# THUDM/GCC

Measured on AMD Instinct MI355X. Metric: sampled-subgraphs/sec, higher is better.
Workload: dtype f32

## Files before the change

### gcc_amd/csrc/posemb.hip

```cpp
#include <mutex>
#include "host_common.h"
#include <type_traits>

namespace {

constexpr int kJMax = GCC_POSEMB_LDS_MAX;
#ifndef GCC_POSEMB_SMALL_T
#define GCC_POSEMB_SMALL_T 256
#endif
constexpr int kSmallT = GCC_POSEMB_SMALL_T;
constexpr int kJSmall = 64;

constexpr int kMaxViews = GCC_POSEMB_MAX_VIEWS;
struct PosView {
    const int32_t *node_off, *row_ptr, *col_idx;
    float *pos, *evals, *raw;
};
struct PosMulti {
    PosView v[kMaxViews];
    int32_t nviews, B, hidden;
    uint64_t seed;
    int32_t *status;
    long long *ticks;
};
// ... 1994 lines not shown
    const int rp0 = a.row_ptr[n0], nnz = a.row_ptr[n0 + n] - rp0;
    const bool csr_lds = nnz <= kCsrCap && nnz < 65536 && n < ldv;
    if (csr_lds) {
        for (int e = tid; e < nnz; e += kKThreads) ccol[e] = (uint16_t)(a.col_idx[rp0 + e] - n0);
        for (int r = tid; r <= n; r += kKThreads) crow[r] = (uint16_t)(a.row_ptr[n0 + r] - rp0);
    }
    __syncthreads();
    const int nl = nlong < kMaxLong ? nlong : kMaxLong;
    const bool long_overflow = nlong > kMaxLong;

    auto orth = [&](int ncols, int hcol) {
        for (int pass = 0; pass < 2; ++pass) {
            for (int i = 2 * wv_id; i < ncols; i += 2 * kKWaves) {
                const float *va = V + (int64_t)i * ldv;
                const bool two = i + 1 < ncols;
                const float *vb = two ? va + ldv : va;
                float a0 = 0.f, a1 = 0.f, b0 = 0.f, b1 = 0.f;
                for (int r = lane; r < n; r += 256) {
                    const int r1 = r + 64, r2 = r + 128, r3 = r + 192;
                    const float x0 = va[r], y0 = vb[r];
                    const float x1 = r1 < n ? va[r1] : 0.f, y1 = r1 < n ? vb[r1] : 0.f;
                    const float x2 = r2 < n ? va[r2] : 0.f, y2 = r2 < n ? vb[r2] : 0.f;
                    const float x3 = r3 < n ? va[r3] : 0.f, y3 = r3 < n ? vb[r3] : 0.f;
                    const float w0 = w[r], w1 = r1 < n ? w[r1] : 0.f, w2 = r2 < n ? w[r2] : 0.f, w3 = r3 < n ? w[r3] : 0.f;
                    a0 = fmaf(x0, w0, a0); a1 = fmaf(x1, w1, a1); a0 = fmaf(x2, w2, a0); a1 = fmaf(x3, w3, a1);
                    b0 = fmaf(y0, w0, b0); b1 = fmaf(y1, w1, b1); b0 = fmaf(y2, w2, b0); b1 = fmaf(y3, w3, b1);
                }
                const float sa = wave_sum(a0 + a1), sb = wave_sum(b0 + b1);
                if (lane == 0) {
                    hbuf[i] = sa;
                    if (two) hbuf[i + 1] = sb;
                }
            }
            __syncthreads();
            if (hcol >= 0 && tid < ncols) H[tid * kM + hcol] += hbuf[tid];
            for (int r = tid; r < n; r += kKThreads) {
                float a0 = w[r], a1 = 0.f, a2 = 0.f, a3 = 0.f;
                int i = 0;
                for (; i + 8 <= ncols; i += 8) {
                    const float v0 = V[(int64_t)i * ldv + r], v1 = V[(int64_t)(i + 1) * ldv + r];
                    const float v2 = V[(int64_t)(i + 2) * ldv + r], v3 = V[(int64_t)(i + 3) * ldv + r];
                    const float v4 = V[(int64_t)(i + 4) * ldv + r], v5 = V[(int64_t)(i + 5) * ldv + r];
                    const float v6 = V[(int64_t)(i + 6) * ldv + r], v7 = V[(int64_t)(i + 7) * ldv + r];
                    a0 = fmaf(-v0, hbuf[i], a0); a1 = fmaf(-v1, hbuf[i + 1], a1);
                    a2 = fmaf(-v2, hbuf[i + 2], a2); a3 = fmaf(-v3, hbuf[i + 3], a3);
                    a0 = fmaf(-v4, hbuf[i + 4], a0); a1 = fmaf(-v5, hbuf[i + 5], a1);
                    a2 = fmaf(-v6, hbuf[i + 6], a2); a3 = fmaf(-v7, hbuf[i + 7], a3);
                }
                for (; i + 4 <= ncols; i += 4) {
                    a0 = fmaf(-V[(int64_t)i * ldv + r], hbuf[i], a0);
                    a1 = fmaf(-V[(int64_t)(i + 1) * ldv + r], hbuf[i + 1], a1);
                    a2 = fmaf(-V[(int64_t)(i + 2) * ldv + r], hbuf[i + 2], a2);
                    a3 = fmaf(-V[(int64_t)(i + 3) * ldv + r], hbuf[i + 3], a3);
                }
                for (; i < ncols; ++i) a0 = fmaf(-V[(int64_t)i * ldv + r], hbuf[i], a0);
                w[r] = (a0 + a1) + (a2 + a3);
            }
            __syncthreads();
        }
    };

    int j = 0, steps = 0, cycle = 0;
    for (; cycle < kMaxCycles; ++cycle) {
        for (; j < kM; ++j, ++steps) {
            for (int r = tid; r < n; r += kKThreads) {
                const int beg = csr_lds ? (int)crow[r] : a.row_ptr[n0 + r] - rp0;
                const int end = csr_lds ? (int)crow[r + 1] : a.row_ptr[n0 + r + 1] - rp0;
                if (end - beg > kLongDeg && !long_overflow) continue;
                float s = 0.f;
                if (csr_lds) for (int e = beg; e < end; ++e) s += x[ccol[e]];
                else for (int e = beg; e < end; ++e) s += x[a.col_idx[rp0 + e] - n0];
                w[r] = s * dinv[r];
            }
            if (!long_overflow) {
                for (int i = wv_id; i < nl; i += kKWaves) {
                    const int r = longrows[i];
                    const int beg = csr_lds ? (int)crow[r] : a.row_ptr[n0 + r] - rp0;
                    const int end = csr_lds ? (int)crow[r + 1] : a.row_ptr[n0 + r + 1] - rp0;
                    float s = 0.f;
                    if (csr_lds) for (int e = beg + lane; e < end; e += 64) s += x[ccol[e]];
                    else for (int e = beg + lane; e < end; e += 64) s += x[a.col_idx[rp0 + e] - n0];
                    s = wave_sum(s);
                    if (lane == 0) w[r] = s * dinv[r];
                }
            }
            __syncthreads();
            orth(j + 1, j);
            float s2 = 0.f;
            for (int r = tid; r < n; r += kKThreads) s2 = fmaf(w[r], w[r], s2);
            float beta = sqrtf(block_sum(s2, red));
            if (beta < 1e-6f) {
                for (int r = tid; r < n; r += kKThreads) {
                    uint32_t rnd[4];
                    philox4x32_10((uint32_t)r, (uint32_t)(steps + 1), (uint32_t)gb, 0x9E0B5EEDu,
                                  (uint32_t)a.seed, (uint32_t)(a.seed >> 32), rnd);
                    w[r] = (float)(rnd[0] >> 8) * (1.0f / 16777216.0f) - 0.5f;
                }
                __syncthreads();
                orth(j + 1, -1);
                float s3 = 0.f;
                for (int r = tid; r < n; r += kKThreads) s3 = fmaf(w[r], w[r], s3);
                nrm = sqrtf(block_sum(s3, red));
                beta = 0.f;
            } else {
                nrm = beta;
            }
            if (tid == 0) H[(j + 1) * kM + j] = beta;
            for (int r = tid; r < n; r += kKThreads) {
                const float vn = w[r] / nrm;
                V[(int64_t)(j + 1) * ldv + r] = vn;
                x[r] = vn * dinv[r];
            }
            __syncthreads();
        }
        PHASE_TICK(0);
        for (int i = tid; i < kM * lda; i += kKThreads) {
            const int r = i / lda, c = i - r * lda;
            float v = 0.f;
            if (c < kM) v = r <= c ? H[r * kM + c] : H[c * kM + r];
            Aj[i] = v;
        }
        __syncthreads();
        tridiagonalize<1, kKThreads, 2>(Aj, lda, kM, tw);
        eig_top_values<kKThreads, kVecCap>(tw, kM, keep, es);
        const bool ritz_failed = eig_top_vectors<1, kKThreads>(Aj, lda, kM, keep, tw, es,
                                                               (uint32_t)a.seed ^ ((uint32_t)gb * 0x9E3779B1u) ^ (uint32_t)cycle,
                                                               nullptr, tick_);
        PHASE_TICK(1);
        if (tid < kM) {
            theta[tid] = tid < keep ? es.lamv[tid] : -2.f;
            sel[tid] = tid < keep ? tid : kM;
        }
        if (tid == 0) { done = 1; flag = ritz_failed ? 2 : 0; }
        __syncthreads();
        const float beta_m = H[kM * kM + (kM - 1)];
        if (tid < k) {
            const float res = fabsf(beta_m * Yj[(kM - 1) * lda + tid]);
            if (res > kRitzTol) done = 0;
            if (res > 10.f * kRitzTol) flag = 2;
        }
        __syncthreads();
        const bool finished = done != 0 || cycle == kMaxCycles - 1;
#ifdef GCC_AMD_HIPEMU
        if (getenv("GCC_POSEMB_DEBUG") && tid == 0) {
            float worst = 0.f; int nbad = 0;
            for (int i = 0; i < kM; ++i) if (sel[i] < k) { const float rs = fabsf(beta_m * Yj[(kM - 1) * lda + i]); worst = rs > worst ? rs : worst; nbad += rs > kRitzTol; }
            fprintf(stderr, "kry b=%d n=%d cycle=%d worst=%.2e nbad=%d theta_k=%.4f\n", b, n, cycle + 1, worst, nbad, 0.f);
        }
#endif
        if (finished && done == 0 && flag == 2 && tid == 0) {
            atomicOr(a.status, (int32_t)GCC_STATUS_POSEMB_NOT_CONVERGED);
            if (atomicAdd(a.status + 4, 1) == 0) { a.status[5] = gb; a.status[6] = kClsKrylov; a.status[7] = n; a.status[8] = -1; a.status[9] = n; }
        }
        if (finished && done == 0 && tid == 0) atomicAdd(a.status + 3, 1);
        const int nout = finished ? k : keep;
        if (tid < kM) {
            const int t = finished ? k - 1 - sel[tid] : sel[tid];
            if (t >= 0 && t < nout) colsrc[t] = tid;
        }
        __syncthreads();
        if (!finished) {
            const int nchunk = (nout + 7) >> 3;
            for (int task = tid; task < n * nchunk; task += kKThreads) {
                const int ch = task / n, r = task - ch * n;
                float acc[8] = {0.f, 0.f, 0.f, 0.f, 0.f, 0.f, 0.f, 0.f};
                int src[8];
#pragma unroll
                for (int u = 0; u < 8; ++u) src[u] = colsrc[min(8 * ch + u, nout - 1)];
                for (int c = 0; c < kM; ++c) {
                    const float v = V[(int64_t)c * ldv + r];
#pragma unroll
                    for (int u = 0; u < 8; ++u) acc[u] = fmaf(v, Yj[c * lda + src[u]], acc[u]);
                }
#pragma unroll
                for (int u = 0; u < 8; ++u)
                    if (8 * ch + u < nout) Valt[(int64_t)(8 * ch + u) * ldv + r] = acc[u];
            }
            for (int r = tid; r < n; r += kKThreads) Valt[(int64_t)keep * ldv + r] = V[(int64_t)kM * ldv + r];
            for (int i = tid; i < (kM + 1) * kM; i += kKThreads) H[i] = 0.f;
            __syncthreads();
            if (tid < kM && sel[tid] < keep) H[sel[tid] * kM + sel[tid]] = theta[tid];
            __syncthreads();
            float *tmp = V; V = Valt; Valt = tmp;
            j = keep;
            PHASE_TICK(2);
            continue;
        }
        float *rawout = a.raw ? a.raw : a.pos;
        const int nchunk = (k + 7) >> 3;
        for (int task = tid; task < n * nchunk; task += kKThreads) {
            const int ch = task / n, r = task - ch * n;
            float acc[8] = {0.f, 0.f, 0.f, 0.f, 0.f, 0.f, 0.f, 0.f};
            int src[8];
#pragma unroll
            for (int u = 0; u < 8; ++u) src[u] = colsrc[min(8 * ch + u, k - 1)];
            for (int c = 0; c < kM; ++c) {
                const float v = V[(int64_t)c * ldv + r];
#pragma unroll
                for (int u = 0; u < 8; ++u) acc[u] = fmaf(v, Yj[c * lda + src[u]], acc[u]);
            }
            float *ro = rawout + (int64_t)(n0 + r) * a.hidden + 8 * ch;
#pragma unroll
            for (int u = 0; u < 8; ++u)
                if (8 * ch + u < k) ro[u] = acc[u];
        }
        __syncthreads();
        for (int r = tid; r < n; r += kKThreads) {
            const float *ro = rawout + (int64_t)(n0 + r) * a.hidden;
            float *po = a.pos + (int64_t)(n0 + r) * a.hidden;
            float s2 = 0.f;
            for (int c = 0; c < k; ++c) s2 = fmaf(ro[c], ro[c], s2);
            const float inv = s2 > 0.f ? 1.0f / sqrtf(s2) : 1.0f;
            for (int c = 0; c < a.hidden; ++c) {
                const float v = c < k ? ro[c] : 0.f;
                po[c] = v * inv;
                if (a.raw) a.raw[(int64_t)(n0 + r) * a.hidden + c] = v;
            }
        }
        if (a.evals && tid < kM && sel[tid] < k) a.evals[(int64_t)b * a.hidden + (k - 1 - sel[tid])] = theta[tid];
        if (a.evals) for (int c = k + tid; c < a.hidden; c += kKThreads) a.evals[(int64_t)b * a.hidden + c] = 0.f;
        break;
    }
    PHASE_TICK(3);
    if (tid == 0) {
        atomicMax(a.status + 1, cycle + 1);
        atomicAdd(a.status + 2, steps);
    }
    }
}


constexpr int kChP = 64;
constexpr int kChPWide = 64, kChPNarrow = 32;
#ifndef GCC_POSEMB_CH_NARROW_WANT
#define GCC_POSEMB_CH_NARROW_WANT 20
#endif
constexpr int kChNarrowWant = GCC_POSEMB_CH_NARROW_WANT;
constexpr int kChNarrowGuards = 8;
#ifndef GCC_POSEMB_CH_THREADS
#define GCC_POSEMB_CH_THREADS 1024
#endif
constexpr int kChThreads = GCC_POSEMB_CH_THREADS;
static_assert(kChThreads % 64 == 0 && kNodeMax % kChThreads == 0 && kChThreads >= 256 && kChThreads <= 1024, "block-class workgroup size");
constexpr int kChRowsPerThread = kNodeMax / kChThreads;
#if defined(GCC_AMD_HIPEMU) || GCC_POSEMB_CH_THREADS > 512
#define GCC_CHEB_REG_CAP
#else
#define GCC_CHEB_REG_CAP __attribute__((amdgpu_waves_per_eu(GCC_POSEMB_CH_THREADS / 256 + 1)))
#endif
constexpr int kChCsrCap = 12288;
#ifndef GCC_POSEMB_CH_LONGDEG
#define GCC_POSEMB_CH_LONGDEG 32
#endif
constexpr int kChLongDeg = GCC_POSEMB_CH_LONGDEG;
constexpr int kChSlabFloats = 4096;
constexpr int kChMaxChunks = kChSlabFloats / 32;
constexpr int kChMaxLong = kChMaxChunks / 2;
constexpr int kChRounds = 16;
constexpr int kChMaxRitz = 5;
constexpr float kChTol = 2e-5f;
constexpr double kChShift = 1e-8;
constexpr float kChAmpLog = 12.9f;
constexpr int kChBw = 32;

struct LdsYes { static constexpr bool value = true; };
struct LdsNo { static constexpr bool value = false; };

constexpr int64_t kChBufFloats = (int64_t)kNodeMax * kChP;
struct ChebArgs {
    PosMulti m;
    PosHead hd;
    float *xws;
    uint32_t *tabs;
};

template <int P>
struct ChebRitzLds {
    static constexpr int Ldy = P + 1;
    static constexpr int Lf = 0;
    static constexpr int Af = Lf + P * Ldy;
    static constexpr int Y = Af + P * Ldy;
    static constexpr int tri = Y + P * Ldy;
    static constexpr int lu = tri + tri_head_floats(P, P * Ldy, kChThreads);
    static constexpr int bytes = (int)sizeof(float) * lu + tri_lu_bytes(P, kChBw);
};
template <int P>
struct ChebDenseLds {
    static constexpr int G = 0, K = G + P * P, Li = K + P * P;
    static constexpr int bytes = (Li + P * P) * (int)sizeof(double);
};
struct ChebLds {
    static constexpr int crow = 0;
    static constexpr int ccol = crow + (int)sizeof(uint16_t) * (kNodeMax + 8);
    static constexpr int scale = ccol + (int)sizeof(uint16_t) * kChCsrCap;
    static constexpr int slab = scale + (int)sizeof(float) * kNodeMax;
    static constexpr int region = slab + (int)sizeof(float) * kChSlabFloats;
    static constexpr int dense_bytes = ChebDenseLds<kChP>::bytes;
    static constexpr int ritz_pad = kChP * (int)sizeof(float);
    static constexpr int ritz_bytes = ChebRitzLds<kChP>::bytes + ritz_pad;
    static constexpr int region_bytes = ritz_bytes > dense_bytes ? ritz_bytes : dense_bytes;
    static constexpr int bytes = region + region_bytes;
    static_assert(region_bytes >= kNodeMax * kDeflNodeBytes, "the deflation tables overlay the region of the dense matrices");
};

__global__ __launch_bounds__(kChThreads) GCC_CHEB_REG_CAP void posemb_cheb_kernel(ChebArgs ca)
{
    DYN_SMEM(smem);
    __shared__ EigShared es;
    __shared__ float theta[kChP], resid[kChP], dsc[kChP];
    __shared__ double dscd[kChP];
    __shared__ int longrow[kChMaxLong], longfirst[kChMaxLong + 1];
    __shared__ int chunk_beg[kChMaxChunks + 1];
    __shared__ uint8_t chunk_row[kChMaxChunks], rowx[kNodeMax];
    __shared__ int sh_clen, sh_long_t;
    __shared__ int wsum[kChThreads / 64 + 1];
    __shared__ int sh_item, sh_tot[3], sh_nlong, sh_nchunk, sh_fail;
    __shared__ int colsrc[64];
    constexpr int kCls = kClsCheb;
    const PosMulti &m = ca.m;
    const PosHead &hd = ca.hd;
    constexpr int kNW = kChThreads / 64;
    uint16_t *crow = (uint16_t *)(smem + ChebLds::crow);
    uint16_t *ccol = (uint16_t *)(smem + ChebLds::ccol);
    float *scale = (float *)(smem + ChebLds::scale);
    float *slab = (float *)(smem + ChebLds::slab);
    unsigned char *region = smem + ChebLds::region;
    for (;;) {
    __syncthreads();
    if (threadIdx.x == 0) sh_item = atomicAdd(hd.next + kCls, 1);
    __syncthreads();
    if (sh_item >= hd.count[kCls]) return;
    uint32_t tid_ = threadIdx.x;
    opaque_u32(tid_);
    const int tid = (int)tid_, lane = tid & 63, wv = tid >> 6;
    const int gb = hd.list[(int64_t)kCls * hd.T + sh_item] & kItemMask;
    PosArgs a;
    int b;
    item_args(m, gb, a, b);
    const int n0 = a.node_off[b], n = a.node_off[b + 1] - n0;
#ifdef GCC_POSEMB_ABLATE_CHEB
    continue;
#endif
    const int k = min(min(n - 2, a.hidden), kMaxVec);
    long long tick_ = m.ticks ? device_ticks() : 0;
    if (m.ticks && tid == 0) atomicAdd((unsigned long long *)&m.ticks[kCls * 16 + 15], 1ull);
    const int32_t *rp = a.row_ptr + n0;
    float *XA0 = ca.xws + (int64_t)blockIdx.x * 3 * kChBufFloats, *XB0 = XA0 + kChBufFloats, *XC0 = XB0 + kChBufFloats;

    Defl d;
    defl_bind(d, region, kNodeMax);
    for (int i = tid; i < n; i += kChThreads) defl_init_node(d, i, rp, a.col_idx, n0);
    if (tid == 0) { sh_fail = 0; sh_nlong = 0; sh_nchunk = 0; }
    __syncthreads();
    for (int i = tid; i < n; i += kChThreads) defl_count_node(d, i, rp, a.col_idx, n0, hd.use_stalks != 0);
    __syncthreads();
    for (int p = tid; p < n; p += kChThreads) defl_order_node(d, p, rp, a.col_idx, n0);
    __syncthreads();
    defl_prefix_block<kChThreads>(d, n, sh_tot, (int *)slab);
    const int nr = sh_tot[0], z = sh_tot[1], zp = sh_tot[2];
    for (int i = tid; i < n; i += kChThreads) {
        if (d.ridx[i] == kNone) continue;
        const int di = rp[i + 1] - rp[i];
        const int pi = d.par[i];
        float sc = 1.0f / sqrtf((float)(di < 1 ? 1 : di));
        if (pi != (int)kNone && d.tcnt[pi] >= 2) {
            sc = sqrtf((float)d.tcnt[pi]);
        } else {
            const int h = d.phub[pi != (int)kNone ? pi : i];
            if (h != (int)kNone && d.pcnt[h] >= 2) sc = pi != (int)kNone ? 1.0f / sqrtf((float)d.pcnt[h]) : sqrtf(0.5f * (float)d.pcnt[h]);
        }
        scale[d.ridx[i]] = sc;
    }
    for (int r = tid; r <= nr; r += kChThreads) crow[r] = 0;
    __syncthreads();
    for (int i = wv; i < n; i += kNW) {
        if (d.ridx[i] == kNone) continue;
        int c = 0;
        for (int e0 = rp[i]; e0 < rp[i + 1]; e0 += 64) {
            const int e = e0 + lane;
            const bool keep = e < rp[i + 1] && d.ridx[a.col_idx[e] - n0] != kNone;
            c += __popcll(wave_ballot(keep));
        }
        if (lane == 0) crow[d.ridx[i] + 1] = (uint16_t)(c > 65535 ? 65535 : c);
    }
    __syncthreads();
    {
        const int r0 = kChRowsPerThread * tid;
        int c[kChRowsPerThread], own = 0;
#pragma unroll
        for (int u = 0; u < kChRowsPerThread; ++u) { c[u] = r0 + u < nr ? (int)crow[r0 + u + 1] : 0; own += c[u]; }
        int incl = wave_scan_incl(own);
        if (lane == 63) wsum[wv] = incl;
        __syncthreads();
        int base = 0;
        for (int q = 0; q < wv; ++q) base += wsum[q];
        incl += base - own;
        __syncthreads();
#pragma unroll
        for (int u = 0; u < kChRowsPerThread; ++u) {
            incl += c[u];
            if (r0 + u < nr) {
                if (incl > kChCsrCap) sh_fail = 1;
                crow[r0 + u + 1] = (uint16_t)(incl > 65535 ? 65535 : incl);
            }
        }
    }
    __syncthreads();
    if (!sh_fail) {
        for (int i = wv; i < n; i += kNW) {
            if (d.ridx[i] == kNone) continue;
            int at = (int)crow[d.ridx[i]];
            for (int e0 = rp[i]; e0 < rp[i + 1]; e0 += 64) {
                const int e = e0 + lane;
                const int rj = e < rp[i + 1] ? (int)d.ridx[a.col_idx[e] - n0] : (int)kNone;
                const unsigned long long mk = wave_ballot(rj != (int)kNone);
                if (rj != (int)kNone) ccol[at + __popcll(mk & lanemask_lt())] = (uint16_t)rj;
                at += __popcll(mk);
            }
        }
    }
    __syncthreads();
    uint16_t *xrec = (uint16_t *)(ca.tabs + (int64_t)blockIdx.x * kTabFloats);
    for (int v = tid; v < n; v += kChThreads) defl_record(d, v, rp, a.col_idx, n0, xrec + 4 * v);
    __syncthreads();
    PHASE_TICK(0);
    bool failed = sh_fail != 0;
    auto build_chunks = [&](int slots) {
        constexpr int R = kChRowsPerThread;
        const int r0 = R * tid;
        int len[R];
#pragma unroll
        for (int u = 0; u < R; ++u) len[u] = (r0 + u < nr && !failed) ? (int)crow[r0 + u + 1] - (int)crow[r0 + u] : 0;
        auto block_scan = [&](int v, int &total) -> int {
            int incl = wave_scan_incl(v);
            if (lane == 63) wsum[wv] = incl;
            __syncthreads();
            int base = 0, tot = 0;
            for (int q = 0; q < kNW; ++q) { if (q < wv) base += wsum[q]; tot += wsum[q]; }
            __syncthreads();
            total = tot;
            return incl - v + base;
        };
        int T = kChLongDeg, nl = 0, x = 0;
        for (;;) {
            int own = 0;
#pragma unroll
            for (int u = 0; u < R; ++u) own += len[u] > T ? 1 : 0;
            x = block_scan(own, nl);
            if (nl <= slots / 2) break;
            T *= 2;
        }
        int own = 0, total = 0;
#pragma unroll
        for (int u = 0; u < R; ++u) own += len[u] > T ? len[u] : 0;
        (void)block_scan(own, total);
        int clen = nl ? (total + (slots - nl) - 1) / (slots - nl) : 8;
        clen = clen < 8 ? 8 : (clen + 3) & ~3;
        own = 0;
#pragma unroll
        for (int u = 0; u < R; ++u) own += len[u] > T ? (len[u] + clen - 1) / clen : 0;
        int nc = 0;
        int fx = block_scan(own, nc);
#pragma unroll
        for (int u = 0; u < R; ++u) {
            const int r = r0 + u;
            const bool lg = len[u] > T;
            if (r < nr) rowx[r] = lg ? (uint8_t)x : (uint8_t)0xFF;
            if (lg) {
                const int nch = (len[u] + clen - 1) / clen;
                longrow[x] = r;
                longfirst[x] = fx;
                for (int j = 0; j < nch; ++j) { chunk_beg[fx + j] = (int)crow[r] + j * clen; chunk_row[fx + j] = (uint8_t)x; }
                ++x;
                fx += nch;
            }
        }
        if (tid == 0) { longfirst[nl] = nc; sh_nlong = nl; sh_nchunk = nc; sh_clen = clen; sh_long_t = T; }
        __syncthreads();
    };
    const int kq = min(k, nr);
    const bool build_failed = failed;
    auto solve = [&](auto pc) -> int {
    constexpr int P = decltype(pc)::value;
    constexpr int Ldy = P + 1;
    constexpr int E = P * P / kChThreads;
    constexpr int TPM = P / E;
    constexpr int TPR = P / 8;
    constexpr int TPQ = P / 4;
    bool failed = build_failed;
    float *XA = XA0, *XB = XB0, *XC = XC0;
    build_chunks(kChSlabFloats / P);
    const int nchunk = sh_nchunk, nlong = sh_nlong, clen = sh_clen, longT = sh_long_t;
#ifdef GCC_AMD_HIPEMU
    if (getenv("GCC_POSEMB_DEBUG") && tid == 0) fprintf(stderr, "cheb item b=%d n=%d nr=%d nnz=%d nlong=%d nchunk=%d fail=%d P=%d clen=%d T=%d\n", b, n, nr, (int)crow[nr], nlong, nchunk, sh_fail, P, clen, longT);
#endif

    constexpr int kChLdsRows = ChebLds::region_bytes / (P * (int)sizeof(float));
    const bool lds_x = nr <= kChLdsRows;
    auto gather = [&](auto in_lds, const float *src, int e0, int e1, float *acc) {
        const float *base = decltype(in_lds)::value ? (const float *)region : src;
        const int q8 = 8 * (tid % TPR);
        for (int e = e0; e < e1; e += 4) {
            int cj[4];
            float sc[4];
            float4 xa[4], xb[4];
#pragma unroll
            for (int u = 0; u < 4; ++u) {
                const bool in = e + u < e1;
                cj[u] = (int)ccol[in ? e + u : e0];
                sc[u] = in ? scale[cj[u]] : 0.f;
            }
#pragma unroll
            for (int u = 0; u < 4; ++u) {
                xa[u] = *(const float4 *)(base + (int64_t)cj[u] * P + q8);
                xb[u] = *(const float4 *)(base + (int64_t)cj[u] * P + q8 + 4);
            }
#pragma unroll
            for (int u = 0; u < 4; ++u) {
                acc[0] = fmaf(sc[u], xa[u].x, acc[0]); acc[1] = fmaf(sc[u], xa[u].y, acc[1]);
                acc[2] = fmaf(sc[u], xa[u].z, acc[2]); acc[3] = fmaf(sc[u], xa[u].w, acc[3]);
                acc[4] = fmaf(sc[u], xb[u].x, acc[4]); acc[5] = fmaf(sc[u], xb[u].y, acc[5]);
                acc[6] = fmaf(sc[u], xb[u].z, acc[6]); acc[7] = fmaf(sc[u], xb[u].w, acc[7]);
            }
        }
    };
    auto spmm_body = [&](auto in_lds, const float *src, float *dst, float alpha, float center, float gamma) {
        const float *base = decltype(in_lds)::value ? (const float *)region : src;
        uint32_t pt_ = (uint32_t)tid;
        opaque_u32(pt_);
        const int q8 = 8 * ((int)pt_ % TPR), g8 = (int)pt_ / TPR;
        auto finish = [&](int r, const float *acc) {
            const float sr = scale[r];
            const float4 oa = *(const float4 *)(base + (int64_t)r * P + q8), ob = *(const float4 *)(base + (int64_t)r * P + q8 + 4);
            float o[8] = {alpha * (sr * acc[0] - center * oa.x), alpha * (sr * acc[1] - center * oa.y),
                          alpha * (sr * acc[2] - center * oa.z), alpha * (sr * acc[3] - center * oa.w),
                          alpha * (sr * acc[4] - center * ob.x), alpha * (sr * acc[5] - center * ob.y),
                          alpha * (sr * acc[6] - center * ob.z), alpha * (sr * acc[7] - center * ob.w)};
            if (gamma != 0.f) {
                const float4 da = *(const float4 *)(dst + (int64_t)r * P + q8), db = *(const float4 *)(dst + (int64_t)r * P + q8 + 4);
                o[0] -= gamma * da.x; o[1] -= gamma * da.y; o[2] -= gamma * da.z; o[3] -= gamma * da.w;
                o[4] -= gamma * db.x; o[5] -= gamma * db.y; o[6] -= gamma * db.z; o[7] -= gamma * db.w;
            }
            *(float4 *)(dst + (int64_t)r * P + q8) = make_float4(o[0], o[1], o[2], o[3]);
            *(float4 *)(dst + (int64_t)r * P + q8 + 4) = make_float4(o[4], o[5], o[6], o[7]);
        };
        for (int c = g8; c < nchunk; c += kChThreads / TPR) {
            const int r = longrow[chunk_row[c]];
            float acc[8] = {0.f, 0.f, 0.f, 0.f, 0.f, 0.f, 0.f, 0.f};
            gather(in_lds, src, chunk_beg[c], min(chunk_beg[c] + clen, (int)crow[r + 1]), acc);
            *(float4 *)(slab + c * P + q8) = make_float4(acc[0], acc[1], acc[2], acc[3]);
            *(float4 *)(slab + c * P + q8 + 4) = make_float4(acc[4], acc[5], acc[6], acc[7]);
        }
        for (int r = g8; r < nr; r += kChThreads / TPR) {
            const int e0 = (int)crow[r], e1 = (int)crow[r + 1];
            if (e1 - e0 > longT) continue;
            float acc[8] = {0.f, 0.f, 0.f, 0.f, 0.f, 0.f, 0.f, 0.f};
            gather(in_lds, src, e0, e1, acc);
            finish(r, acc);
        }
        if (nchunk) {
            __syncthreads();
            for (int x = g8; x < nlong; x += kChThreads / TPR) {
                float acc[8] = {0.f, 0.f, 0.f, 0.f, 0.f, 0.f, 0.f, 0.f};
                for (int c = longfirst[x]; c < longfirst[x + 1]; ++c) {
                    const float4 pa = *(const float4 *)(slab + c * P + q8), pb = *(const float4 *)(slab + c * P + q8 + 4);
                    acc[0] += pa.x; acc[1] += pa.y; acc[2] += pa.z; acc[3] += pa.w;
                    acc[4] += pb.x; acc[5] += pb.y; acc[6] += pb.z; acc[7] += pb.w;
                }
                finish(longrow[x], acc);
            }
        }
        __syncthreads();
    };
    constexpr int RPP = kChThreads / TPR;
    constexpr int kPasses = kChLdsRows / RPP;
    static_assert(kChLdsRows == kPasses * RPP, "an LDS-resident block is covered in kPasses passes");
    auto filter_step_lds = [&](float *prev, float alpha, float center, float gamma) {
        float *xs = (float *)region;
        uint32_t pt_ = (uint32_t)tid;
        opaque_u32(pt_);
        const int q8 = 8 * ((int)pt_ % TPR), g8 = (int)pt_ / TPR;
        float nw[kPasses][8];
        auto finish = [&](int ps, int r, const float *acc) {
            float4 da = make_float4(0.f, 0.f, 0.f, 0.f), db = da;
            float *pr_ = prev + (int64_t)r * P + q8;
            if (gamma != 0.f) { da = *(const float4 *)pr_; db = *(const float4 *)(pr_ + 4); }
            const float sr = scale[r];
            const float4 oa = *(const float4 *)(xs + r * P + q8), ob = *(const float4 *)(xs + r * P + q8 + 4);
            nw[ps][0] = alpha * (sr * acc[0] - center * oa.x) - gamma * da.x; nw[ps][1] = alpha * (sr * acc[1] - center * oa.y) - gamma * da.y;
            nw[ps][2] = alpha * (sr * acc[2] - center * oa.z) - gamma * da.z; nw[ps][3] = alpha * (sr * acc[3] - center * oa.w) - gamma * da.w;
            nw[ps][4] = alpha * (sr * acc[4] - center * ob.x) - gamma * db.x; nw[ps][5] = alpha * (sr * acc[5] - center * ob.y) - gamma * db.y;
            nw[ps][6] = alpha * (sr * acc[6] - center * ob.z) - gamma * db.z; nw[ps][7] = alpha * (sr * acc[7] - center * ob.w) - gamma * db.w;
            *(float4 *)pr_ = oa;
            *(float4 *)(pr_ + 4) = ob;
        };
        for (int c = g8; c < nchunk; c += RPP) {
            const int r = longrow[chunk_row[c]];
            float acc[8] = {0.f, 0.f, 0.f, 0.f, 0.f, 0.f, 0.f, 0.f};
            gather(LdsYes(), xs, chunk_beg[c], min(chunk_beg[c] + clen, (int)crow[r + 1]), acc);
            *(float4 *)(slab + c * P + q8) = make_float4(acc[0], acc[1], acc[2], acc[3]);
            *(float4 *)(slab + c * P + q8 + 4) = make_float4(acc[4], acc[5], acc[6], acc[7]);
        }
#pragma unroll
        for (int ps = 0; ps < kPasses; ++ps) {
            const int r = g8 + ps * RPP;
            if (r < nr) {
                const int e0 = (int)crow[r], e1 = (int)crow[r + 1];
                if (e1 - e0 <= longT) {
                    float acc[8] = {0.f, 0.f, 0.f, 0.f, 0.f, 0.f, 0.f, 0.f};
                    gather(LdsYes(), xs, e0, e1, acc);
                    finish(ps, r, acc);
                }
            }
        }
        if (nchunk) {
            __syncthreads();
#pragma unroll
            for (int ps = 0; ps < kPasses; ++ps) {
                const int r = g8 + ps * RPP;
                if (r < nr && rowx[r] != 0xFF) {
                    const int x = rowx[r];
                    float acc[8] = {0.f, 0.f, 0.f, 0.f, 0.f, 0.f, 0.f, 0.f};
                    for (int c = longfirst[x]; c < longfirst[x + 1]; ++c) {
                        const float4 pa = *(const float4 *)(slab + c * P + q8), pb = *(const float4 *)(slab + c * P + q8 + 4);
                        acc[0] += pa.x; acc[1] += pa.y; acc[2] += pa.z; acc[3] += pa.w;
                        acc[4] += pb.x; acc[5] += pb.y; acc[6] += pb.z; acc[7] += pb.w;
                    }
                    finish(ps, r, acc);
                }
            }
        }
        __syncthreads();
#pragma unroll
        for (int ps = 0; ps < kPasses; ++ps) {
            const int r = g8 + ps * RPP;
            if (r < nr) {
                *(float4 *)(xs + r * P + q8) = make_float4(nw[ps][0], nw[ps][1], nw[ps][2], nw[ps][3]);
                *(float4 *)(xs + r * P + q8 + 4) = make_float4(nw[ps][4], nw[ps][5], nw[ps][6], nw[ps][7]);
            }
        }
        __syncthreads();
    };
    auto spmm = [&](const float *src, float *dst, float alpha, float center, float gamma) {
        if (lds_x) {
            float4 *xs = (float4 *)region;
            const float4 *gs = (const float4 *)src;
            for (int i = tid; i < nr * (P / 4); i += kChThreads) xs[i] = gs[i];
            __syncthreads();
            spmm_body(LdsYes(), src, dst, alpha, center, gamma);
        } else {
            spmm_body(LdsNo(), src, dst, alpha, center, gamma);
        }
    };

    using Dense = ChebDenseLds<P>;
    double *G = (double *)region + Dense::G, *K = (double *)region + Dense::K;
    float cut = 0.2f;
    int deg = 6, remaining = 6, round = 0, nrr = 0;
    unsigned long long flops = 0;
    const unsigned long long nnz_ = (unsigned long long)crow[nr], nr_ = (unsigned long long)nr;
    bool converged = false;
    if (!failed) {
        for (int i = tid; i < nr * P; i += kChThreads)
            XA[i] = hash_unit((uint32_t)a.seed ^ ((uint32_t)gb * 0x9E3779B1u), (uint32_t)(i & (P - 1)), (uint32_t)(i / P));
        __syncthreads();
    }
    for (; round < kChRounds && !failed; ++round) {
        uint32_t rt_ = (uint32_t)tid;
        opaque_u32(rt_);
        const int tid = (int)rt_, lane = tid & 63, wv = tid >> 6;
        const int mi = tid / TPM, mj = E * (tid % TPM);
        remaining -= deg;
#ifdef GCC_AMD_HIPEMU
        if (getenv("GCC_POSEMB_RR_ALWAYS")) remaining = 0;
#endif
        const bool rr = remaining <= 0;
        const bool vals_only = rr && nrr == 0, fullrr = rr && !vals_only;
        if (lds_x && !(hd.use_cheb & 4)) {
            const float e = 0.5f * (cut + 1.0f), cen = 0.5f * (cut - 1.0f);
            float sigma = e / (1.0f - cen);
            const float tau = 2.0f / sigma;
            float4 *xs = (float4 *)region;
            for (int i = tid; i < nr * (P / 4); i += kChThreads) xs[i] = ((const float4 *)XA)[i];
            __syncthreads();
            filter_step_lds(XB, sigma / e, cen, 0.f);
            for (int i = 2; i <= deg; ++i) {
                const float sn = 1.0f / (tau - sigma);
                filter_step_lds(XB, 2.0f * sn / e, cen, sigma * sn);
                sigma = sn;
            }
            for (int i = tid; i < nr * (P / 4); i += kChThreads) ((float4 *)XA)[i] = xs[i];
            if (rr) spmm_body(LdsYes(), XA, XB, 1.0f, 0.f, 0.f);
            else __syncthreads();
        } else {
            const float e = 0.5f * (cut + 1.0f), cen = 0.5f * (cut - 1.0f);
            float sigma = e / (1.0f - cen);
            const float tau = 2.0f / sigma;
            spmm(XA, XB, sigma / e, cen, 0.f);
            float *prev = XA, *cur = XB;
            for (int i = 2; i <= deg; ++i) {
                const float sn = 1.0f / (tau - sigma);
                spmm(cur, prev, 2.0f * sn / e, cen, sigma * sn);
                float *t = prev; prev = cur; cur = t;
                sigma = sn;
            }
            if (rr) spmm(XA, XB, 1.0f, 0.f, 0.f);
        }
        flops += (unsigned long long)(deg + (rr ? 1 : 0)) * (2ull * nnz_ * P + 5ull * nr_ * P)
                 + (rr ? 2ull : 1ull) * 2ull * nr_ * P * P + 2ull * P * P * P
                 + (rr ? 4ull * P * P * P : 0ull) + (fullrr ? 2ull : 1ull) * 2ull * nr_ * P * P;
        PHASE_TICK(1);
// ... 699 lines not shown
```

Before: 717,700.

## Stage subgraph edges in LDS and build deflation order and CSR edge-parallel

Copies the subgraph's edge list into LDS as local column/row pairs, using a binary search over a staged row pointer to find each edge's row. Deflation ordering, kept-row counts and compacted CSR columns are then computed edge-parallel with wave ballots, per-chunk tail counts and cross-chunk prefix sums, replacing the per-node and per-row wave loops. The aim is to spread work evenly when degrees are skewed and to avoid repeated global col_idx reads. In exchange it adds extra passes, barriers, LDS atomics and binary searches, and it only applies when the entry count fits the staging capacity.

Result: no change. 724,900, median of 6 (+1.0%).

```diff
diff --git a/gcc_amd/csrc/posemb.hip b/gcc_amd/csrc/posemb.hip
--- a/gcc_amd/csrc/posemb.hip
+++ b/gcc_amd/csrc/posemb.hip
@@ -2320,6 +2320,18 @@
     static constexpr int bytes = region + region_bytes;
     static_assert(region_bytes >= kNodeMax * kDeflNodeBytes, "the deflation tables overlay the region of the dense matrices");
 };
+struct ChebStage {
+    static constexpr int srp = kNodeMax * kDeflNodeBytes;
+    static constexpr int cnt = srp + (int)sizeof(uint16_t) * (kNodeMax + 8);
+    static constexpr int tails = cnt + (int)sizeof(int) * kNodeMax;
+    static constexpr int chunks = (ChebLds::region_bytes - tails) / (4 * 64 + 6);
+    static constexpr int cap = 64 * chunks;
+    static constexpr int col = tails + 3 * (int)sizeof(uint16_t) * chunks;
+    static constexpr int row = col + (int)sizeof(uint16_t) * cap;
+    static_assert(chunks > 0 && row + (int)sizeof(uint16_t) * cap <= ChebLds::region_bytes, "the staged entries fit behind the deflation tables");
+    static_assert(cap < 65536, "entry offsets are uint16");
+    static_assert(cap == 16448, "the staging bound stated above and in tests/test_posemb_matrix_build_emu.py");
+};
 
 __global__ __launch_bounds__(kChThreads) GCC_CHEB_REG_CAP void posemb_cheb_kernel(ChebArgs ca)
 {
@@ -2367,12 +2379,82 @@
 
     Defl d;
     defl_bind(d, region, kNodeMax);
+    const int ebase = rp[0], nent = rp[n] - ebase;
+    const bool staged = nent <= ChebStage::cap && !(hd.use_cheb & 8);
+    uint16_t *srp = (uint16_t *)(region + ChebStage::srp), *tails = (uint16_t *)(region + ChebStage::tails);
+    uint16_t *scol = (uint16_t *)(region + ChebStage::col), *srow = (uint16_t *)(region + ChebStage::row);
+    int *rcnt = (int *)(region + ChebStage::cnt);
+    auto stage_tails = [&](int ta, int tb, auto mark) {
+        for (int e0 = 64 * wv; e0 < nent; e0 += kChThreads) {
+            const int e = e0 + lane;
+            const bool valid = e < nent;
+            const int p = valid ? (int)srow[e] : 0, j = valid ? (int)scol[e] : 0;
+            bool fa = false, fb = false;
+            if (valid) mark(p, j, fa, fb);
+            const unsigned long long ma = wave_ballot(fa), mb = wave_ballot(fb);
+            const int plast = wave_readlane(p, min(64, nent - e0) - 1);
+            const int s = max(0, (int)srp[plast] - e0);
+            if (lane == 0) {
+                tails[ta * ChebStage::chunks + (e0 >> 6)] = (uint16_t)__popcll(ma & (~0ull << s));
+                if (tb != ta) tails[tb * ChebStage::chunks + (e0 >> 6)] = (uint16_t)__popcll(mb & (~0ull << s));
+            }
+        }
+    };
+    auto stage_ranks = [&](int ta, int tb, auto mark, auto use) {
+        for (int e0 = 64 * wv; e0 < nent; e0 += kChThreads) {
+            const int e = e0 + lane;
+            const bool valid = e < nent;
+            const int p = valid ? (int)srow[e] : 0, j = valid ? (int)scol[e] : 0;
+            bool fa = false, fb = false;
+            if (valid) mark(p, j, fa, fb);
+            const unsigned long long ma = wave_ballot(fa), mb = wave_ballot(fb);
+            const int p0 = wave_readlane(p, 0);
+            int ca = 0, cb = 0;
+            for (int c = ((int)srp[p0] >> 6) + lane; c < (e0 >> 6); c += 64) {
+                ca += (int)tails[ta * ChebStage::chunks + c];
+                cb += (int)tails[tb * ChebStage::chunks + c];
+            }
+            ca = wave_last(wave_scan_incl(ca));
+            cb = wave_last(wave_scan_incl(cb));
+            if (fa || fb) {
+                const int s = (int)srp[p] - e0;
+                const unsigned long long below = lanemask_lt() & (~0ull << max(0, s));
+                use(p, j, fa, fb, __popcll((fa ? ma : mb) & below) + (s < 0 ? (fa ? ca : cb) : 0));
+            }
+        }
+    };
+    auto mark_groups = [&](int p, int j, bool &ft, bool &fs) {
+        ft = d.tcnt[p] >= 2 && d.par[j] == (uint16_t)p;
+        fs = !ft && d.pcnt[p] >= 2 && d.phub[j] == (uint16_t)p;
+    };
+    auto mark_kept = [&](int p, int j, bool &fk, bool &) { fk = d.ridx[p] != kNone && d.ridx[j] != kNone; };
     for (int i = tid; i < n; i += kChThreads) defl_init_node(d, i, rp, a.col_idx, n0);
+    if (staged)
+        for (int i = tid; i <= n; i += kChThreads) srp[i] = (uint16_t)(rp[i] - ebase);
     if (tid == 0) { sh_fail = 0; sh_nlong = 0; sh_nchunk = 0; }
     __syncthreads();
     for (int i = tid; i < n; i += kChThreads) defl_count_node(d, i, rp, a.col_idx, n0, hd.use_stalks != 0);
-    __syncthreads();
-    for (int p = tid; p < n; p += kChThreads) defl_order_node(d, p, rp, a.col_idx, n0);
+    if (staged)
+        for (int e = tid; e < nent; e += kChThreads) {
+            scol[e] = (uint16_t)(a.col_idx[ebase + e] - n0);
+            int lo = 0, hi = n;
+            while (hi - lo > 1) {
+                const int mid = (lo + hi) >> 1;
+                if ((int)srp[mid] <= e) lo = mid; else hi = mid;
+            }
+            srow[e] = (uint16_t)lo;
+        }
+    __syncthreads();
+    if (staged) {
+        stage_tails(0, 1, mark_groups);
+        __syncthreads();
+        stage_ranks(0, 1, mark_groups, [&](int p, int j, bool ft, bool, int o) {
+            if (o == 0) (ft ? d.rep : d.prep)[p] = (uint16_t)j;
+            d.ord[j] = (uint16_t)o;
+        });
+    } else {
+        for (int p = tid; p < n; p += kChThreads) defl_order_node(d, p, rp, a.col_idx, n0);
+    }
     __syncthreads();
     defl_prefix_block<kChThreads>(d, n, sh_tot, (int *)slab);
     const int nr = sh_tot[0], z = sh_tot[1], zp = sh_tot[2];
@@ -2389,8 +2471,24 @@
         }
         scale[d.ridx[i]] = sc;
     }
-    for (int r = tid; r <= nr; r += kChThreads) crow[r] = 0;
-    __syncthreads();
+    for (int r = tid; r <= nr; r += kChThreads) { crow[r] = 0; if (staged && r < nr) rcnt[r] = 0; }
+    __syncthreads();
+    if (staged) {
+        stage_tails(2, 2, mark_kept);
+        for (int e0 = 64 * wv; e0 < nent; e0 += kChThreads) {
+            const int e = e0 + lane;
+            const bool valid = e < nent;
+            const int p = valid ? (int)srow[e] : 0, j = valid ? (int)scol[e] : 0;
+            bool fk = false, unused = false;
+            if (valid) mark_kept(p, j, fk, unused);
+            const unsigned long long mk = wave_ballot(fk);
+            const int s = max(0, (int)srp[p] - e0), t = min(64, (int)srp[p + 1] - e0);
+            if (valid && lane == s && d.ridx[p] != kNone) {
+                const int c = __popcll(mk & (~0ull << s) & (t == 64 ? ~0ull : (1ull << t) - 1ull));
+                if (c) atomicAdd(&rcnt[d.ridx[p]], c);
+            }
+        }
+    } else
     for (int i = wv; i < n; i += kNW) {
         if (d.ridx[i] == kNone) continue;
         int c = 0;
@@ -2406,7 +2504,10 @@
         const int r0 = kChRowsPerThread * tid;
         int c[kChRowsPerThread], own = 0;
 #pragma unroll
-        for (int u = 0; u < kChRowsPerThread; ++u) { c[u] = r0 + u < nr ? (int)crow[r0 + u + 1] : 0; own += c[u]; }
+        for (int u = 0; u < kChRowsPerThread; ++u) {
+            c[u] = r0 + u < nr ? (staged ? min(rcnt[r0 + u], 65535) : (int)crow[r0 + u + 1]) : 0;
+            own += c[u];
+        }
         int incl = wave_scan_incl(own);
         if (lane == 63) wsum[wv] = incl;
         __syncthreads();
@@ -2424,7 +2525,9 @@
         }
     }
     __syncthreads();
-    if (!sh_fail) {
+    if (!sh_fail && staged) {
+        stage_ranks(2, 2, mark_kept, [&](int p, int j, bool, bool, int o) { ccol[(int)crow[d.ridx[p]] + o] = d.ridx[j]; });
+    } else if (!sh_fail) {
         for (int i = wv; i < n; i += kNW) {
             if (d.ridx[i] == kNone) continue;
             int at = (int)crow[d.ridx[i]];
```
